# ruchikachavhan/diffusion-models-moe

Hardware: AMD Instinct MI355X
Metric: images/sec SD-1.4 512² 50-step DDIM, expert mask on; 1→8 GPU scaling (higher is better)
Workload: dtype fp16; 1 GPU; SD-1.4 MoE-fied (relu, top-k 0.2, expert 20) + RemoveExperts skilled-expert mask, 512^2 (4x64x64 latents), 50 DDIM steps, CFG 7.5; prompts_per_gpu=8, global_batch=8, parallelism=dp1

## Files before the change

diffusion-models-moe_amd/sdmoe/_lib.py:

```python
from __future__ import annotations

import ctypes
import os

_HERE = os.path.dirname(os.path.abspath(__file__))
LIB_PATH = os.path.join(_HERE, "libsdmoe_hip.so")

_P = ctypes.c_void_p
_L = ctypes.c_long
_I = ctypes.c_int
_F = ctypes.c_float
_FP = ctypes.POINTER(ctypes.c_float)
_IP = ctypes.POINTER(ctypes.c_int)

SIGNATURES = {
    "sdmoe_linear": [_P, _L, _P, _L, _P, _P, _L, _I, _P, _L, _P, _L, _I, _I, _I, _I, _P, _L, _P],
    "sdmoe_conv3x3": [_P, _L, _I, _I, _I, _I, _P, _P, _P, _L, _P, _L, _P, _L, _I, _I, _I, _I, _P, _L, _P],
    "sdmoe_conv3x3_sc": [_P, _L, _I, _I, _I, _I, _P, _P, _P, _L, _P, _L, _I, _P, _L, _I, _I, _P, _L, _P],
    "sdmoe_conv3x3_gn": [_P, _L, _I, _I, _I, _I, _P, _P, _I, _P, _P, _P, _L, _P, _L, _P, _L, _I, _P, _L, _I, _P, _L,
                         _P],
    "sdmoe_conv_up2x": [_P, _L, _I, _I, _I, _I, _P, _P, _P, _L, _I, _P, _L, _P],
    "sdmoe_conv_up2x_plan": [_I, _I, _I, _I, _I, _L, _P],
    "sdmoe_groupnorm_apply": [_P, _L, _I, _I, _I, _P, _P, _I, _P, _L, _P],
    "sdmoe_mask_weight": [_P, _P, _L, _L, _P, _P],
    "sdmoe_groupnorm_stats": [_P, _L, _I, _I, _I, _I, _P, _P, _F, _P, _P, _P, _L, _P],
    "sdmoe_groupnorm": [_P, _L, _I, _I, _I, _I, _P, _P, _F, _I, _P, _L, _P, _P, _P, _L, _P],
    "sdmoe_gn_fold": [_P, _L, _I, _I, _P, _P, _P, _I, _P, _P, _P],
    "sdmoe_linear_per_image": [_P, _L, _P, _L, _L, _P, _L, _I, _P, _L, _P, _L, _I, _I, _I, _P, _L, _P],
    "sdmoe_layernorm": [_P, _L, _P, _L, _I, _I, _P, _P, _F, _P],
    "sdmoe_ln_fold": [_P, _L, _I, _I, _P, _P, _P, _P, _L, _P, _P, _P],
    "sdmoe_linear_ln": [_P, _L, _P, _L, _P, _P, _F, _P, _L, _I, _I, _I, _P],
    "sdmoe_linear_geglu_ln": [_P, _L, _P, _L, _P, _P, _F, _P, _L, _I, _I, _I, _I, _P, _L, _I, _P],
    "sdmoe_attention": [_P, _L, _P, _L, _P, _L, _P, _L, _I, _I, _I, _I, _I, _F, _P],
    "sdmoe_geglu_route": [_P, _L, _I, _I, _I, _I, _I, _P, _P, _P, _P, _P, _L, _P, _L, _P, _P, _P],
    "sdmoe_score_bias": [_P, _L, _I, _I, _P, _P, _L, _P],
    "sdmoe_geglu_route_bias": [_P, _L, _I, _I, _I, _I, _I, _P, _P, _P, _P, _P, _L, _P, _L, _P, _P, _P, _P],
    "sdmoe_linear_geglu": [_P, _L, _P, _L, _P, _P, _L, _I, _I, _I, _I, _P, _L, _I, _P],
    "sdmoe_moe_topk_mask": [_P, _L, _I, _I, _I, _I, _I, _P, _L, _P, _P, _P],
    "sdmoe_moe_topk_keep": [_I, _I, _I, _I, _I, _P, _L, _P, _P, _P, _P],
    "sdmoe_linear_keep": [_P, _L, _P, _P, _L, _P, _P, _L, _P, _L, _I, _I, _I, _P, _L, _P],
    "sdmoe_linear_masked": [_P, _L, _P, _P, _L, _P, _P, _P, _L, _P, _L, _I, _I, _I, _P, _L, _P],
    "sdmoe_linear_masked_sets": [_P, _L, _P, _P, _L, _P, _L, _P, _I, _I, _P, _P, _L, _P, _L, _I, _I, _I, _P, _L, _P],
    "sdmoe_gemm_plan_sets": [_I, _I, _I, _I, _I, _I, _L, _P],
    "sdmoe_wmask_union_sets": [_P, _L, _I, _P, _I, _L, _P, _P],
    "sdmoe_gemm_plan": [_I, _I, _I, _I, _I, _I, _L, _P],
    "sdmoe_conv_plan": [_I, _I, _I, _I, _I, _I, _I, _I, _I, _I, _I, _L, _P],
    "sdmoe_wmask_kmajor": [_P, _L, _I, _I, _P, _P, _P],
    "sdmoe_timestep_embedding": [_P, _P, _F, _I, _I, _F, _P],
    "sdmoe_cfg_multistep_step": [_P, _L, _P, _I, _I, _I, _F, _P, _P, _P, _P, _P, _L, _P],
    "sdmoe_sqdist_f32": [_P, _L, _P, _L, _I, _I, _I, _P, _L, _P],
    "sdmoe_balanced_assign": [_P, _I, _I, ctypes.c_double, _P, _I, _P],
    "sdmoe_expert_mean_topk": [_P, _L, _I, _I, _I, _P, _I, _I, _P, _P, _P, _L, _P],
    "sdmoe_colnorm_accum": [_P, _L, _I, _I, _P, _P, _L, _P],
    "sdmoe_wanda_mask": [_P, _L, _I, _I, _P, _P, _I, _P, _P],
    "sdmoe_union_over_time": [_P, _L, _I, _L, _F, _P, _P],
    "sdmoe_geglu_neurons": [_P, _L, _I, _I, _I, _P, _F, _P, _L, _P, _L, _I, _P, _I, _P, _P, _P, _L, _P],
    "sdmoe_expert_stats": [_P, _L, _P, _I, _I, _I, _P, _I, _P, _P, _P, _L, _P],
    "sdmoe_geglu_sparsity": [_P, _L, _I, _I, _I, _F, _P, _L, _P, _L, _I, _P, _I, _P, _P, _P, _P, _L, _P],
    "sdmoe_noise_capture": [_P, _L, _P, _L, _L, _P],
    "sdmoe_noise_distance": [_P, _L, _L, _P, _L, _L, _I, _I, _I, _P, _I, _P, _P, _L, _P],
    "sdmoe_clip_quantise": [_P, _I, _I, _I, _I, _P, _P],
    "sdmoe_clip_resample_h": [_P, _L, _I, _I, _I, _I, _I, _P, _P, _I, _I, _P, _P],
    "sdmoe_clip_resample_v": [_P, _I, _I, _I, _P, _P, _I, _I, _I, _FP, _FP, _P, _P, _L, _I, _P],
    "sdmoe_clip_scores": [_P, _L, _P, _L, _P, _L, _I, _I, _P, _P],
    "sdmoe_text_pool": [_P, _L, _I, _I, _I, _I, _I, _P, _L, _P],
    "sdmoe_concept_route": [_P, _L, _I, _I, _I, _P, _L, _I, _P, _P, _I, _P, _P, _P, _P],
    "sdmoe_softmax_rows": [_P, _L, _P, _L, _I, _I, _P],
    "sdmoe_transpose": [_P, _L, _P, _L, _I, _I, _P],
    "sdmoe_gather_rows": [_P, _L, _P, _I, _I, _P, _L, _I, _P, _L, _P],
    "sdmoe_attention_short": [_P, _L, _P, _L, _P, _L, _P, _L, _I, _I, _I, _I, _F, _I, _P],
    "sdmoe_timestep_embedding_rows": [_P, _L, _P, _I, _I, _I, _I, _F, _P],
    "sdmoe_prepare_input": [_P, _P, _I, _I, _L, _I, _P],
    "sdmoe_cfg_ddim_step": [_P, _L, _P, _I, _I, _I, _F, _F, _F, _P, _L, _P],
    "sdmoe_cfg_x0_step": [_P, _L, _P, _I, _I, _I, _F, _P, _P, _P, _P, _L, _P],
    "sdmoe_prepare_input_scaled": [_P, _P, _I, _I, _L, _I, _F, _F, _P],
    "sdmoe_add": [_P, _P, _P, _L, _P],
    "sdmoe_tune": [_I, _I],
    "sdmoe_tune_knob": [_I, _IP, ctypes.POINTER(ctypes.c_char_p), _IP, _IP],
    "sdmoe_tune_reset": [],
    "sdmoe_set_gelu_table": [_P],
    "sdmoe_version": [],
}

ERRORS = {-1: "bad pointer/size", -2: "unsupported shape/alignment", -3: "unsupported mode"}

_lib = None


class SdmoeError(RuntimeError):
    pass


def load(path: str | None = None):
    global _lib
    if _lib is not None:
        return _lib
    p = path or os.environ.get("SDMOE_LIB", LIB_PATH)
    if not os.path.exists(p):
        raise SdmoeError(
            f"libsdmoe_hip.so not found at {p}: build it with `python -c 'import __graft_entry__ as g; g.build()'` "
            "(or `make -C diffusion-models-moe_amd/csrc`). There is no CPU fallback."
        )
    lib = ctypes.CDLL(p)
    ab_lib = os.environ.get("SDMOE_AB", "0") == "1"
    for name, argt in SIGNATURES.items():
        if ab_lib and not hasattr(lib, name):
            continue
        fn = getattr(lib, name)
        fn.argtypes = argt
        fn.restype = ctypes.c_char_p if name == "sdmoe_version" else ctypes.c_int
    for k, v in parse_tune(os.environ.get("SDMOE_TUNE", ""), lib):
        check(lib.sdmoe_tune(k, v), f"sdmoe_tune({k}={v})")
    _lib = lib
    return lib

# ... 42 lines not shown
```

diffusion-models-moe_amd/sdmoe/ops.py:

```python
from __future__ import annotations

import ctypes
import os

import torch

from . import _lib

ACT_NONE, ACT_SILU, ACT_GELU, ACT_RELU, ACT_QUICK_GELU = 0, 1, 2, 3, 4
ACT_BY_NAME = {"none": ACT_NONE, "silu": ACT_SILU, "gelu": ACT_GELU, "relu": ACT_RELU, "quick_gelu": ACT_QUICK_GELU}


_raw_stream = getattr(torch._C, "_cuda_getCurrentRawStream", None)
_cur_dev = getattr(torch._C, "_cuda_getDevice", None)


def _stream():
    if _raw_stream is not None and _cur_dev is not None:
        return _raw_stream(_cur_dev())
    return torch.cuda.current_stream().cuda_stream


def _ptr(t):
    return None if t is None else t.data_ptr()
# ... 492 lines not shown
    lib = _lib.load()
    xp, lda = _rows(x, "x")
    M, K = x.shape
    nimg, N, Kw = wf.shape
    if Kw != K or M != nimg * rows_per_batch or tuple(colbias.shape) != (nimg, N):
        raise ValueError(f"linear_per_image: x {tuple(x.shape)}, wf {tuple(wf.shape)}, colbias "
                         f"{tuple(colbias.shape)}, rows_per_batch {rows_per_batch}")
    if out is None:
        out = torch.empty((M, N), dtype=torch.float16, device=x.device)
    op, ldc = _rows(out, "out")
    rp, ldr = (None, 0) if residual is None else _rows(residual, "residual")
    ws = _workspace(x.device)
    st = lib.sdmoe_linear_per_image(xp, lda, _dev(wf, "wf"), wf.stride(1), wf.stride(0),
                                    _dev(colbias, "colbias", torch.float32), colbias.stride(0), rows_per_batch, rp,
                                    ldr, op, ldc, M, N, K, ws.data_ptr(), ws.numel(), _stream())
    _lib.check(st, "sdmoe_linear_per_image")
    return out


def layernorm(x, gamma, beta, eps=1e-5, out=None):
    lib = _lib.load()
    xp, ldx = _rows(x, "x")
    M, C = x.shape
    if out is None:
        out = torch.empty((M, C), dtype=torch.float16, device=x.device)
    op, ldy = _rows(out, "out")
    st = lib.sdmoe_layernorm(xp, ldx, op, ldy, M, C, _dev(gamma, "gamma"), _dev(beta, "beta"), float(eps), _stream())
    _lib.check(st, "sdmoe_layernorm")
    return out


class LNFold:

    def __init__(self, w, gamma, beta, eps, bias=None):
        lib = _lib.load()
        N, K = w.shape
        self.eps = float(eps)
        self.w = torch.empty((N, K), dtype=torch.float16, device=w.device)
        self.bias = torch.empty(N, dtype=torch.float32, device=w.device)
        self.wsum = torch.empty(N, dtype=torch.float32, device=w.device)
        if bias is not None:
            _dev(bias, "bias")
        st = lib.sdmoe_ln_fold(_dev(w, "w"), w.stride(0), N, K, _dev(gamma, "gamma"), _dev(beta, "beta"), _ptr(bias),
                               self.w.data_ptr(), K, self.bias.data_ptr(), self.wsum.data_ptr(), _stream())
        _lib.check(st, "sdmoe_ln_fold")

    def rows(self, idx):
        f = LNFold.__new__(LNFold)
        f.eps, f.w, f.bias, f.wsum = self.eps, self.w[idx].contiguous(), self.bias[idx].contiguous(), \
            self.wsum[idx].contiguous()
        return f


def linear_ln(x, fold: LNFold, out=None):
    lib = _lib.load()
    xp, lda = _rows(x, "x")
    M, K = x.shape
    N = fold.w.shape[0]
    if fold.w.shape[1] != K:
        raise ValueError(f"linear_ln: folded weight {tuple(fold.w.shape)} does not match input K={K}")
    if out is None:
        out = torch.empty((M, N), dtype=torch.float16, device=x.device)
    op, ldc = _rows(out, "out")
    st = lib.sdmoe_linear_ln(xp, lda, fold.w.data_ptr(), fold.w.stride(0), fold.bias.data_ptr(), fold.wsum.data_ptr(),
                             fold.eps, op, ldc, M, N, K, _stream())
    _lib.check(st, "sdmoe_linear_ln")
    return out


def attention(q, k, v, nimg, Nq, Nk, heads, out=None, scale=None):
    lib = _lib.load()
    qp, ldq = _rows(q, "q")
    kp, ldk = _rows(k, "k")
    vp, ldv = _rows(v, "v")
    C = q.shape[1]
    d = C // heads
    if out is None:
        out = torch.empty((nimg * Nq, C), dtype=torch.float16, device=q.device)
    op, ldo = _rows(out, "out")
    if scale is None:
        scale = d ** -0.5
    st = lib.sdmoe_attention(qp, ldq, kp, ldk, vp, ldv, op, ldo, nimg, Nq, Nk, heads, d, float(scale), _stream())
    _lib.check(st, "sdmoe_attention")
    return out


class Routing:

    def __init__(self, labels: torch.Tensor, num_experts: int, k: int, device):
        labels = labels.to(torch.int64).cpu()
        F = labels.numel()
        if labels.min() < 0 or labels.max() >= num_experts:
            raise ValueError("expert labels out of range")
        order = torch.argsort(labels, stable=True)
        counts = torch.bincount(labels, minlength=num_experts)
        off = torch.zeros(num_experts + 1, dtype=torch.int64)
        off[1:] = torch.cumsum(counts, 0)
        self.F, self.E, self.k = F, int(num_experts), int(k)
        self.labels = labels.to(torch.int32).to(device)
        self.e_off = off.to(torch.int32).to(device)
        self.e_nid = order.to(torch.int32).to(device)
        sizes = set(counts.tolist())
        self.esize = sizes.pop() if len(sizes) == 1 else 0
        self.perm = order
        self.perm_dev = order.to(torch.int32).to(device)
        self.fusable = bool(self.esize and 40 % self.esize == 0 and F % 80 == 0 and self.E <= 256)

    @classmethod
    def from_patterns(cls, patterns: torch.Tensor, k: int, device=None):
        p = patterns.detach().float().cpu()
        E, F = p.shape
        if not torch.all((p == 0) | (p == 1)) or not torch.all(p.sum(0) == 1):
            raise ValueError("patterns must be a 0/1 [E, F] matrix with exactly one expert per neuron")
        labels = p.argmax(0)
        return cls(labels, E, k, device or patterns.device)


def geglu_rows(F: int, perm: torch.Tensor | None, device) -> torch.Tensor:
    if F % 2:
        raise ValueError(f"GEGLU layout: F = {F} is odd")
    idx = torch.arange(F, device=device) if perm is None else perm.to(device)
    r = torch.arange(2 * F, device=device)
    q, e = r // 4, r % 4
    c = 2 * q + (e & 1)
    return torch.where(e < 2, idx[c], F + idx[c])


def interleave_geglu(weight: torch.Tensor, bias: torch.Tensor | None, perm: torch.Tensor | None):
    F2, K = weight.shape
    rows = geglu_rows(F2 // 2, perm, weight.device)
    b = torch.zeros(F2, dtype=weight.dtype, device=weight.device) if bias is None else bias
    return weight[rows].contiguous(), b[rows].contiguous()


def interleave_ln_fold(fold: LNFold, perm: torch.Tensor | None) -> LNFold:
    F = fold.w.shape[0] // 2
    return fold.rows(geglu_rows(F, perm, fold.w.device))


_GELU_TABLES = {}


def gelu_table_values() -> torch.Tensor:
    i = torch.arange(16384, dtype=torch.int32)
    bits = (0x2800 + (i & 8191)) | ((i >> 13) << 15)
    return bits.to(torch.int16).view(torch.float16)


def ensure_gelu_table(device) -> torch.Tensor:
    dev = torch.device(device)
    idx = dev.index if dev.index is not None else torch.cuda.current_device()
    t = _GELU_TABLES.get(idx)
    if t is None:
        t = torch.nn.functional.gelu(gelu_table_values().to(torch.device("cuda", idx))).contiguous()
        lib = _lib.load()
        if _lib.has(lib, "sdmoe_set_gelu_table"):
            with torch.cuda.device(idx):
                _lib.check(lib.sdmoe_set_gelu_table(t.data_ptr()), "sdmoe_set_gelu_table")
        _GELU_TABLES[idx] = t
    return t


def linear_geglu(x, w_il, b_il, act=ACT_GELU, *, score=None, esize=0, out=None, ln: LNFold | None = None):
    lib = _lib.load()
    if act == ACT_GELU:
        ensure_gelu_table(x.device)
# ... 762 lines not shown
```

diffusion-models-moe_amd/sdmoe/unet.py:

```python
from __future__ import annotations

import os

import torch
import torch.nn as nn
import torch.nn.functional as F

from . import ops
from .config import UNetConfig

CTX_LEN = 77
FUSED_GEGLU = True
FUSED_KEEP = True
FUSED_LN = os.environ.get("SDMOE_FUSED_LN", "1") != "0"
FUSED_LN_FFN = os.environ.get("SDMOE_FUSED_LN_FFN", "0") == "1"
FUSED_SC = os.environ.get("SDMOE_FUSED_SC", "1") != "0"
FUSED_GN = os.environ.get("SDMOE_FUSED_GN", "1") != "0"
GN_FOLD_MIN_HW = 1024
UPCONV_COLLAPSE = os.environ.get("SDMOE_UPCONV_COLLAPSE", "1") != "0"
IN_PAD = 64
OUT_PAD = 8


def _buf(t):
    return nn.Parameter(t, requires_grad=False)


class LoRACompatibleLinear(nn.Module):

    def __init__(self, weight, bias=None):
        super().__init__()
        self.weight = _buf(weight)
        self.bias = None if bias is None else _buf(bias)
        self._sdmoe_deferred = 0

    @property
    def in_features(self):
        return self.weight.shape[1]

    @property
    def out_features(self):
        return self.weight.shape[0]

    def run(self, x2d, weight=None, **kw):
        return ops.linear(x2d, self.weight if weight is None else weight, self.bias, **kw)

    def forward(self, x, scale=1.0):
        if self._sdmoe_deferred and self._forward_hooks:
            return None
        shp = x.shape
        return self.run(x.reshape(-1, shp[-1])).view(*shp[:-1], self.out_features)


class Conv2d(nn.Module):

    def __init__(self, weight, bias, stride=1):
        super().__init__()
        self.weight = _buf(weight)
        self.bias = _buf(bias)
        self.stride = stride


class Norm(nn.Module):
    def __init__(self, weight, bias, eps, groups=None):
        super().__init__()
        self.weight = _buf(weight)
        self.bias = _buf(bias)
        self.eps = eps
        self.groups = groups

    def stats(self, x2d, nimg, HW):
        return ops.groupnorm_stats(x2d, nimg, HW, self.weight, self.bias, self.eps, self.groups)

    def normalize(self, x2d, nimg, HW, silu):
        return ops.groupnorm(x2d, nimg, HW, self.weight, self.bias, self.eps, self.groups, silu)


def act_code(fn):
    from_name = getattr(fn, "_sdmoe_act", None)
    if from_name is not None:
        return ops.ACT_BY_NAME[from_name]
    if fn is F.gelu or fn is torch.nn.functional.gelu:
        return ops.ACT_GELU
    if fn is F.relu or fn is torch.relu:
        return ops.ACT_RELU
    raise NotImplementedError(f"GEGLU activation {fn!r} has no HIP kernel (supported: gelu, relu)")


def _gelu(x):
    return F.gelu(x)


_gelu._sdmoe_act = "gelu"


class GEGLU(nn.Module):

    def __init__(self, proj: LoRACompatibleLinear):
        super().__init__()
        self.proj = proj
        self.gelu = _gelu
        self.patterns = None
# ... 150 lines not shown
        return view(out), view(gate)

    def sparsity(self, x, threshold=0.0, col_zero=None, col_neg=None, totals=None, img_group=None, ngroups=1,
                 want_gate=False):
        y, rpi, gate, view = self._seam_operands(x, want_gate)
        out = ops.geglu_sparsity(y, act_code(self.gelu), threshold=threshold, rows_per_img=rpi, img_group=img_group,
                                 ngroups=ngroups, col_zero=col_zero, col_neg=col_neg, totals=totals, gate_out=gate)
        return view(out), view(gate)

    def forward(self, x, scale=1.0):
        if self._sdmoe_deferred and self._forward_hooks:
            return None
        return self.routed(x)[0]


def _sole_receiver(module, method):
    hooks = list(module._forward_hooks.values())
    if len(hooks) != 1:
        return None
    owner = getattr(hooks[0], "__self__", None)
    if owner is None or not getattr(owner, "_sdmoe_receiver", False) or not hasattr(owner, method):
        return None
    return owner


def _ln_safe_hook(module, owner):
    if owner is None:
        return False
    hooks = list(module._forward_hooks.values())
    fn = getattr(hooks[0], "__func__", None) if len(hooks) == 1 else None
    return fn is not None and fn is getattr(type(owner), "_sdmoe_ln_safe_hook", None)


class FeedForward(nn.Module):
    def __init__(self, geglu, down):
        super().__init__()
        self.net = nn.ModuleList([geglu, nn.Dropout(0.0), down])
        self._wperm_key = None
        self._wperm = None

    def _down_weight_permuted(self, routing):
        w = self.net[2].weight
        key = (id(routing), w.data_ptr(), w._version)
        if self._wperm_key != key:
            self._wperm = w.data[:, routing.perm.to(w.device)].contiguous()
            self._wperm_key = key
        return self._wperm

    def run(self, x2d, nimg, residual, ln=None):
        geglu, down = self.net[0], self.net[2]
        dhooks = bool(down._forward_hooks)
        masker = _sole_receiver(down, "fused_linear") if dhooks else None
        owner = _sole_receiver(geglu, "hook_fn") if geglu._forward_hooks else None
        geglu._allow_permuted_out = (not dhooks or masker is not None) and (not geglu._forward_hooks or owner is not None)
        if ln is not None and geglu._forward_hooks and not _ln_safe_hook(geglu, owner):
            x2d = ops.layernorm(x2d, ln.weight, ln.bias, ln.eps)
            ln = None
        xv = x2d.view(nimg, -1, x2d.shape[1])
        geglu._ln_pending = (xv, ln) if ln is not None else None
        try:
            h = geglu(xv)
        finally:
            geglu._allow_permuted_out = False
            geglu._ln_pending = None
        h2 = h.reshape(-1, h.shape[-1])
        perm = geglu._out_perm
        permuted = perm is not None and perm[1] == h2.data_ptr()
        if dhooks and not (permuted and masker is not None):
            o = down(h)
            return ops.add(o.reshape(residual.shape).contiguous(), residual)
        if permuted:
            wp = self._down_weight_permuted(perm[0])
            keep = geglu._out_keep
            keep = keep[0] if keep is not None and keep[1] == h2.data_ptr() else None
            if masker is not None:
                kw = {"nimg": nimg} if getattr(masker, "_sdmoe_fused_nimg", False) else {}
                return masker.fused_linear(down, h2, keep, perm[0].perm_dev, wp, residual, **kw)
            if keep is not None:
                return ops.linear_keep(h2, keep, wp, down.bias, residual=residual)
            return ops.linear(h2, wp, down.bias, residual=residual)
        return down.run(h2, residual=residual)


class Attention(nn.Module):
    def __init__(self, wq, wk, wv, wo, bo, heads, self_attn):
        super().__init__()
        self.heads = heads
        self.self_attn = self_attn
        C = wq.shape[0]
        if self_attn:
            self.w_qkv = _buf(torch.cat([wq, wk, wv], 0).contiguous())
            self.to_q = LoRACompatibleLinear(self.w_qkv.data[:C])
            self.to_k = LoRACompatibleLinear(self.w_qkv.data[C:2 * C])
            self.to_v = LoRACompatibleLinear(self.w_qkv.data[2 * C:])
        else:
            self.w_kv = _buf(torch.cat([wk, wv], 0).contiguous())
            self.to_q = LoRACompatibleLinear(wq)
            self.to_k = LoRACompatibleLinear(self.w_kv.data[:C])
            self.to_v = LoRACompatibleLinear(self.w_kv.data[C:])
        self.to_out = nn.ModuleList([LoRACompatibleLinear(wo, bo), nn.Dropout(0.0)])
        self._kv_key = None
        self._kv = None
        self._ln_key = None
        self._ln_fold = None

    def _fold(self, norm):
        w = self.w_qkv if self.self_attn else self.to_q.weight
        key = (w.data_ptr(), w._version, norm.weight.data_ptr(), norm.weight._version, norm.bias.data_ptr(),
               norm.bias._version)
        if self._ln_key != key:
            self._ln_fold = ops.LNFold(w.data, norm.weight.data, norm.bias.data, norm.eps)
            self._ln_key = key
        return self._ln_fold

    def cross_kv(self, ctx2d):
        key = (ctx2d, ctx2d._version, self.w_kv.data_ptr(), self.w_kv._version)
        k = self._kv_key
        if k is None or k[0] is not ctx2d or k[1:] != key[1:]:
            self._kv = ops.linear(ctx2d, self.w_kv)
            self._kv_key = key
        return self._kv

    def run(self, x2d, nimg, N, residual, ctx2d=None, ln=None):
        C = x2d.shape[1]
        if self.self_attn:
            qkv = ops.linear(x2d, self.w_qkv) if ln is None else ops.linear_ln(x2d, self._fold(ln))
            a = ops.attention(qkv[:, :C], qkv[:, C:2 * C], qkv[:, 2 * C:], nimg, N, N, self.heads)
        else:
            q = ops.linear(x2d, self.to_q.weight) if ln is None else ops.linear_ln(x2d, self._fold(ln))
            kv = self.cross_kv(ctx2d)
            a = ops.attention(q, kv[:, :C], kv[:, C:], nimg, N, ctx2d.shape[0] // nimg, self.heads)
        return self.to_out[0].run(a, residual=residual)


class BasicTransformerBlock(nn.Module):
    def __init__(self, norm1, attn1, norm2, attn2, norm3, ff):
        super().__init__()
        self.norm1, self.attn1, self.norm2, self.attn2, self.norm3, self.ff = norm1, attn1, norm2, attn2, norm3, ff

    def run(self, hs, nimg, N, ctx2d):
        if FUSED_LN and hs.shape[1] % 64 == 0:
            hs = self.attn1.run(hs, nimg, N, residual=hs, ln=self.norm1)
            hs = self.attn2.run(hs, nimg, N, residual=hs, ctx2d=ctx2d, ln=self.norm2)
            if FUSED_LN_FFN:
                return self.ff.run(hs, nimg, residual=hs, ln=self.norm3)
            n = ops.layernorm(hs, self.norm3.weight, self.norm3.bias, self.norm3.eps)
            return self.ff.run(n, nimg, residual=hs)
        n = ops.layernorm(hs, self.norm1.weight, self.norm1.bias, self.norm1.eps)
        hs = self.attn1.run(n, nimg, N, residual=hs)
        n = ops.layernorm(hs, self.norm2.weight, self.norm2.bias, self.norm2.eps)
        hs = self.attn2.run(n, nimg, N, residual=hs, ctx2d=ctx2d)
        n = ops.layernorm(hs, self.norm3.weight, self.norm3.bias, self.norm3.eps)
        return self.ff.run(n, nimg, residual=hs)


class Transformer2DModel(nn.Module):

    def __init__(self, norm, proj_in, blocks, proj_out):
        super().__init__()
        self.norm = norm
        self.proj_in = proj_in
        self.transformer_blocks = nn.ModuleList(blocks)
        self.proj_out = proj_out

    def run(self, x, nimg, HW, ctx2d, out):
        pi = self.proj_in
        if FUSED_GN and HW >= GN_FOLD_MIN_HW and HW % 256 == 0 and x.shape[1] % 64 == 0 and not pi._forward_hooks:
            scale, shift = self.norm.stats(x, nimg, HW)
            wf, cb = ops.gn_fold(pi.weight, pi.bias, scale, shift)
            hs = ops.linear_per_image(x, wf, cb, HW)
        else:
            hs = pi.run(self.norm.normalize(x, nimg, HW, False))
        for blk in self.transformer_blocks:
            hs = blk.run(hs, nimg, HW, ctx2d)
        return self.proj_out.run(hs, residual=x, out=out)


class ResnetBlock2D(nn.Module):
    def __init__(self, norm1, conv1, temb_proj, norm2, conv2, shortcut):
        super().__init__()
        self.norm1, self.conv1, self.time_emb_proj, self.norm2, self.conv2 = norm1, conv1, temb_proj, norm2, conv2
        self.conv_shortcut = shortcut
        self.temb_slice = None
        self._sc_key = None
        self._sc_w = None

    def _conv2_with_shortcut(self):
        w2, b2, ws, bs = self.conv2.weight, self.conv2.bias, self.conv_shortcut.weight, self.conv_shortcut.bias
        key = tuple(None if t is None else (t.data_ptr(), t._version) for t in (w2, b2, ws, bs))
        if self._sc_key != key:
            b = sum(t.data.float() for t in (b2, bs) if t is not None)
            self._sc_w = (ops.conv_weight_with_shortcut(w2.data, ws.data),
                          None if isinstance(b, int) else b.half())
            self._sc_key = key
        return self._sc_w

    def run(self, x, nimg, H, W, temb_all, out):
        HW = H * W
        o, n = self.temb_slice
        bstride = temb_all.stride(0) if temb_all.shape[0] > 1 else 0
        cmid = self.conv1.weight.shape[0]
        if ops.conv_gn_fusable(H, W, x.shape[1], cmid):
            h = ops.conv3x3(x, nimg, H, W, self.conv1.weight, self.conv1.bias, coladd=temb_all[:, o:o + n],
                            coladd_bstride=bstride, gn=self.norm1.stats(x, nimg, HW) + (True,))
        else:
            xn = self.norm1.normalize(x, nimg, HW, True)
            h = ops.conv3x3(xn, nimg, H, W, self.conv1.weight, self.conv1.bias,
                            coladd=temb_all[:, o:o + n], coladd_bstride=bstride)
        gn2 = None
        hn = h
        if ops.conv_gn_fusable(H, W, cmid, self.conv2.weight.shape[0]):
            gn2 = self.norm2.stats(h, nimg, HW) + (True,)
        else:
# ... 297 lines not shown
```

include/sdmoe.h:

```cpp
#ifndef SDMOE_H
#define SDMOE_H

#ifdef __cplusplus
extern "C" {
#endif

#define SDMOE_ACT_NONE 0
#define SDMOE_ACT_SILU 1
#define SDMOE_ACT_GELU 2
#define SDMOE_ACT_RELU 3
#define SDMOE_ACT_QUICK_GELU 4

const char* sdmoe_version(void);

int sdmoe_linear(const void* A, long lda, const void* W, long ldw, const void* bias, const void* coladd,
                 long coladd_bstride, int rows_per_batch, const void* R, long ldr, void* C, long ldc, int M, int N,
                 int K, int act, float* workspace, long workspace_floats, void* stream);

int sdmoe_conv3x3(const void* X, long ldx, int nimg, int H, int W, int Cin, const void* Wt, const void* bias,
                  const void* coladd, long coladd_bstride, const void* R, long ldr, void* Y, long ldy, int Cout,
                  int stride, int upsample, int act, float* workspace, long workspace_floats, void* stream);

int sdmoe_conv3x3_sc(const void* X, long ldx, int nimg, int H, int W, int Cin, const void* Wt, const void* bias,
                     const void* coladd, long coladd_bstride, const void* X2, long ldx2, int Cin2, void* Y, long ldy,
                     int Cout, int act, float* workspace, long workspace_floats, void* stream);

int sdmoe_conv3x3_gn(const void* X, long ldx, int nimg, int H, int W, int Cin, const float* gn_scale,
                     const float* gn_shift, int silu, const void* Wt, const void* bias, const void* coladd,
                     long coladd_bstride, const void* R, long ldr, const void* X2, long ldx2, int Cin2, void* Y,
                     long ldy, int Cout, float* workspace, long workspace_floats, void* stream);

int sdmoe_conv_up2x(const void* X, long ldx, int nimg, int H, int W, int Cin, const void* Wc, const void* bias, void* Y,
                    long ldy, int Cout, float* workspace, long workspace_floats, void* stream);
int sdmoe_conv_up2x_plan(int nimg, int H, int W, int Cin, int Cout, long workspace_floats, int* out);

int sdmoe_groupnorm_apply(const void* X, long ldx, int nimg, int HW, int C, const float* scale, const float* shift,
                          int silu, void* Y, long ldy, void* stream);

int sdmoe_mask_weight(const void* W, const void* bits, long N, long K, void* Wm, void* stream);

int sdmoe_groupnorm_stats(const void* X, long ldx, int nimg, int HW, int C, int groups, const void* gamma,
                          const void* beta, float eps, float* scale, float* shift, float* workspace,
                          long workspace_floats, void* stream);

int sdmoe_groupnorm(const void* X, long ldx, int nimg, int HW, int C, int groups, const void* gamma, const void* beta,
                    float eps, int silu, void* Y, long ldy, float* scale, float* shift, float* workspace,
                    long workspace_floats, void* stream);

int sdmoe_gn_fold(const void* W, long ldw, int N, int K, const void* bias, const float* scale, const float* shift,
                  int nimg, void* Wf, float* colbias, void* stream);
int sdmoe_linear_per_image(const void* A, long lda, const void* Wf, long ldw, long w_bstride, const float* colbias,
                           long colbias_bstride, int rows_per_batch, const void* R, long ldr, void* C, long ldc, int M,
                           int N, int K, float* workspace, long workspace_floats, void* stream);

int sdmoe_layernorm(const void* X, long ldx, void* Y, long ldy, int M, int C, const void* gamma, const void* beta,
                    float eps, void* stream);

int sdmoe_ln_fold(const void* W, long ldw, int N, int K, const void* gamma, const void* beta, const void* bias,
                  void* Wf, long ldf, float* bias_f, float* wsum, void* stream);
int sdmoe_linear_ln(const void* A, long lda, const void* Wf, long ldw, const float* bias_f, const float* wsum,
                    float eps, void* C, long ldc, int M, int N, int K, void* stream);
int sdmoe_linear_geglu_ln(const void* A, long lda, const void* W, long ldw, const float* bias_f, const float* wsum,
                          float eps, void* P, long ldp, int M, int F, int K, int act, void* score, long ld_score,
                          int esize, void* stream);

int sdmoe_attention(const void* Q, long ldq, const void* K, long ldk, const void* V, long ldv, void* O, long ldo,
                    int nimg, int Nq, int Nk, int heads, int head_dim, float scale, void* stream);

int sdmoe_geglu_route(const void* Y, long ldy, int M, int F, int E, int k, int act, const int* labels,
                      const int* e_off, const int* e_nid, const unsigned* removed_bits, void* out, long ldo,
                      void* gate_out, long ldg, unsigned* sel_out, void* score_out, void* stream);

int sdmoe_score_bias(const void* score, long ld_score, int M, int E, const void* bias, void* out, long ld_out,
                     void* stream);
int sdmoe_geglu_route_bias(const void* Y, long ldy, int M, int F, int E, int k, int act, const int* labels,
                           const int* e_off, const int* e_nid, const unsigned* removed_bits, void* out, long ldo,
                           void* gate_out, long ldg, unsigned* sel_out, void* score_out, const void* bias,
                           void* stream);

int sdmoe_linear_geglu(const void* A, long lda, const void* W, long ldw, const void* bias, void* P, long ldp,
                       int M, int F, int K, int act, void* score, long ld_score, int esize, void* stream);
int sdmoe_moe_topk_mask(void* P, long ldp, int M, int F, int E, int esize, int k, const void* score,
                        long ld_score, const unsigned* removed_bits, unsigned* sel_out, void* stream);

int sdmoe_moe_topk_keep(int M, int F, int E, int esize, int k, const void* score, long ld_score,
                        const unsigned* removed_bits, void* keep, unsigned* sel_out, void* stream);
int sdmoe_linear_keep(const void* A, long lda, const void* keep, const void* W, long ldw, const void* bias,
                      const void* R, long ldr, void* C, long ldc, int M, int N, int K, float* workspace,
                      long workspace_floats, void* stream);

int sdmoe_linear_masked(const void* A, long lda, const void* keep, const void* W, long ldw, const void* wmask,
                        const void* bias, const void* R, long ldr, void* C, long ldc, int M, int N, int K,
                        float* workspace, long workspace_floats, void* stream);

int sdmoe_linear_masked_sets(const void* A, long lda, const void* keep, const void* W, long ldw, const void* wmasks,
                             long set_stride, const int* image_set, int nsets, int rows_per_img, const void* bias,
                             const void* R, long ldr, void* C, long ldc, int M, int N, int K, float* workspace,
                             long workspace_floats, void* stream);

int sdmoe_gemm_plan_sets(int has_keep, int M, int N, int K, int rows_per_img, int has_residual, long workspace_floats,
                         int* out);

int sdmoe_wmask_union_sets(const void* masks, long mask_stride, int nconcepts, const unsigned* select, int nsets,
                           long words, void* out, void* stream);

int sdmoe_gemm_plan(int mode, int M, int N, int K, int has_residual, int act, long workspace_floats, int* out);

int sdmoe_conv_plan(int nimg, int H, int W, int Cin, int Cin2, int Cout, int stride, int upsample, int has_residual,
                    int gn, int act, long workspace_floats, int* out);

int sdmoe_wmask_kmajor(const void* bits, long ldb, int N, int K, const int* perm, void* out, void* stream);

int sdmoe_expert_mean_topk(const void* score, long ld_score, int M, int E, int rows_per_img, const int* row_idx,
                           int n_idx, int k, void* mean_out, int* topk_out, float* workspace, long workspace_floats,
                           void* stream);
int sdmoe_expert_stats(const void* score, long ld_score, const unsigned* sel, int M, int E, int rows_per_img,
                       const int* img_group, int ngroups, void* colmax, int* count, float* workspace,
                       long workspace_floats, void* stream);
int sdmoe_colnorm_accum(const void* P, long ldp, int M, int F, float* sumsq, float* workspace, long workspace_floats,
                        void* stream);
int sdmoe_wanda_mask(const void* W, long ldw, int C, int F, const void* norm_base, const void* norm_adj, int kprune,
                     void* bits, void* stream);

int sdmoe_geglu_neurons(const void* Y, long ldy, int M, int F, int act, const unsigned* override_bits,
                        float override_value, void* out, long ldo, void* gate_out, long ldg, int rows_per_img,
                        const int* img_group, int ngroups, const unsigned* pos_bits, void* colmax, float* workspace,
                        long workspace_floats, void* stream);

int sdmoe_geglu_sparsity(const void* Y, long ldy, int M, int F, int act, float threshold, void* out, long ldo,
                         void* gate_out, long ldg, int rows_per_img, const int* img_group, int ngroups, int* col_zero,
                         int* col_neg, int64_t* totals, float* workspace, long workspace_floats, void* stream);

int sdmoe_sqdist_f32(const float* X, long ldx, const float* C, long ldc, int n, int k, int d, float* D, long ldd,
                     void* stream);
int sdmoe_balanced_assign(const double* cost, int n, int k, double scale, int64_t* prices, int warm, int* labels);

int sdmoe_union_over_time(const void* bits, long t_stride_bytes, int T, long nbytes, float threshold, void* out,
                          void* stream);

int sdmoe_softmax_rows(const void* X, long ldx, void* Y, long ldy, int R, int N, void* stream);
int sdmoe_transpose(const void* X, long ldx, void* Y, long ldy, int R, int C, void* stream);

int sdmoe_gather_rows(const void* table, long ld_table, const int* idx, int R, int C, const void* add, long ld_add,
                      int period, void* out, long ld_out, void* stream);
int sdmoe_attention_short(const void* Q, long ldq, const void* K, long ldk, const void* V, long ldv, void* O,
                          long ldo, int nseq, int N, int heads, int head_dim, float scale, int causal, void* stream);

int sdmoe_timestep_embedding(void* out, const float* t_dev, float t, int dim, int flip_sin_to_cos, float freq_shift,
                             void* stream);
int sdmoe_timestep_embedding_rows(void* out, long ldo, const float* t_dev, int n, int group, int dim,
// ... 58 lines not shown
```

Baseline: 9.810 images/s.

## Fuse LN-folded Q projection, cross-attention and output projection into one kernel

Adds a single HIP kernel for the C=320, 8-head cross-attention block. Each 128-row tile computes the LayerNorm statistics, the folded Q GEMM, per-head attention over up to 96 keys, the output projection with bias, and the residual add, all kept in LDS. Weight slabs and K/V are triple/double-buffered through LDS with async buffer loads. This removes the Q and attention-output round trips through global memory and two extra launches. The cost is heavy LDS use that allows only one block per CU, and the path is limited to one specific shape with a fallback to the old path otherwise.

```diff
diff --git a/diffusion-models-moe_amd/csrc/xattn_block.hip b/diffusion-models-moe_amd/csrc/xattn_block.hip
--- /dev/null
+++ b/diffusion-models-moe_amd/csrc/xattn_block.hip
@@ -0,0 +1,385 @@
+#include <type_traits>
+
+#include "common.h"
+#include "../../include/sdmoe.h"
+
+namespace {
+
+constexpr int C = 320, HEADS = 8, D = 40;
+constexpr int BM = 128, NW = 8, NT = NW * 64;
+constexpr int XRS = 336;
+constexpr int KSTEP = 32, NKS = C / KSTEP;
+constexpr int SLAB = C * KSTEP;
+constexpr int NPIECE = SLAB * 2 / 1024;
+constexpr int MAXK = 96;
+constexpr int KVROWS = 128;
+constexpr int RS = 48, SL = RS / 8, CH = D / 8;
+constexpr int KVT = KVROWS * RS;
+constexpr int KVPIECE = KVT * 2 / 1024;
+constexpr int SLOT = 2 * KVT;
+constexpr unsigned OOB = 0x80000000u;
+static_assert(2 * KVPIECE == 3 * NW, "three K/V pieces per wave and head");
+static_assert(SLAB <= SLOT, "a slab fits a ring slot");
+
+struct XParams {
+  const half_t* x; long ldx;
+  const half_t* wq; long ldwq; const float* bq; const float* wsum; float eps;
+  const half_t* K; long ldk; const half_t* V; long ldv; int Nk;
+  const half_t* wo; long ldwo; const half_t* bo;
+  half_t* out; long ldo;
+  int Nq;
+  float scale_log2;
+};
+
+SDMOE_DEV half4 ds_read_tr(const half_t* p) {
+  typedef short s4 __attribute__((ext_vector_type(4)));
+  s4 v = __builtin_amdgcn_ds_read_tr16_b64_v4i16((s4 __attribute__((address_space(3)))*)(p));
+  return __builtin_bit_cast(half4, v);
+}
+
+SDMOE_DEV float max3(float a, float b, float c) { return fmaxf(fmaxf(a, b), c); }
+SDMOE_DEV float max2(float a, float b) { return fmaxf(a, b); }
+SDMOE_DEV float max_xrows(float v) {
+  auto r = __builtin_amdgcn_permlane32_swap(__float_as_uint(v), __float_as_uint(v), false, false);
+  v = max2(__uint_as_float(r[0]), __uint_as_float(r[1]));
+  auto t = __builtin_amdgcn_permlane16_swap(__float_as_uint(v), __float_as_uint(v), false, false);
+  return max2(__uint_as_float(t[0]), __uint_as_float(t[1]));
+}
+
+typedef __attribute__((address_space(3))) void lds_void_t;
+SDMOE_DEV void bld16(__amdgpu_buffer_rsrc_t rs, const half_t* lds_dst, unsigned voff) {
+  __builtin_amdgcn_raw_ptr_buffer_load_lds(rs, (lds_void_t*)lds_dst, 16, voff, 0, 0, 0);
+}
+template <int N>
+SDMOE_DEV void vm_wait() { asm volatile("s_waitcnt vmcnt(%0)" ::"n"(N) : "memory"); }
+SDMOE_DEV void barrier() {
+  __builtin_amdgcn_s_barrier();
+  asm volatile("" ::: "memory");
+}
+
+SDMOE_DEV int swz(int t) { return (0x78 >> (2 * t)) & 3; }
+
+__global__ __launch_bounds__(NT, 1) void xattn_block_kernel(XParams p) {
+  __shared__ __attribute__((aligned(1024))) half_t XT[BM * XRS];
+  __shared__ __attribute__((aligned(1024))) half_t R0[SLOT];
+  __shared__ __attribute__((aligned(1024))) half_t R1[SLOT];
+  __shared__ __attribute__((aligned(1024))) half_t R2[SLOT];
+  __shared__ __attribute__((aligned(1024))) half_t ONES[16 * 16];
+  __shared__ float LNROW[BM * 2];
+
+  const int tid = threadIdx.x, lane = tid & 63;
+  const int wave = __builtin_amdgcn_readfirstlane(tid >> 6);
+  const int g = lane >> 4, w = lane & 15;
+  const int wr = wave >> 2, wc = wave & 3;
+  const int tile = xcd_remap(blockIdx.x, gridDim.x);
+  const long row0 = (long)tile * BM;
+  const int img = (int)(row0 / p.Nq);
+
+  const __amdgpu_buffer_rsrc_t rsWq = __builtin_amdgcn_make_buffer_rsrc(
+      (void*)p.wq, (short)0, (int)((C - 1) * p.ldwq * 2 + C * 2), 0x00020000);
+  const __amdgpu_buffer_rsrc_t rsWo = __builtin_amdgcn_make_buffer_rsrc(
+      (void*)p.wo, (short)0, (int)((C - 1) * p.ldwo * 2 + C * 2), 0x00020000);
+  const __amdgpu_buffer_rsrc_t rsK = __builtin_amdgcn_make_buffer_rsrc(
+      (void*)(p.K + (long)img * p.Nk * p.ldk), (short)0, (int)(((long)p.Nk - 1) * p.ldk * 2 + C * 2), 0x00020000);
+  const __amdgpu_buffer_rsrc_t rsV = __builtin_amdgcn_make_buffer_rsrc(
+      (void*)(p.V + (long)img * p.Nk * p.ldv), (short)0, (int)(((long)p.Nk - 1) * p.ldv * 2 + C * 2), 0x00020000);
+
+  auto slot_at = [&](int i) -> half_t* { return i == 0 ? R0 : (i == 1 ? R1 : R2); };
+
+  const int wrow = lane >> 2, wchunk = (lane & 3) ^ swz((lane >> 4) & 3);
+  auto issue_slab = [&](__amdgpu_buffer_rsrc_t rs, long ldw, int ks, half_t* dst) {
+#pragma unroll
+    for (int j = 0; j < 3; ++j) {
+      const int pc = wave + NW * j;
+      if (j < 2 || wave < NPIECE - 2 * NW)
+        bld16(rs, dst + pc * 512, (unsigned)((16 * pc + wrow) * ldw * 2 + wchunk * 16 + ks * (KSTEP * 2)));
+    }
+  };
+
+  float4v acc[4][5];
+  const int aoff = w * KSTEP + ((g ^ swz((w >> 2) & 3)) << 3);
+  auto tile_gemm = [&](__amdgpu_buffer_rsrc_t rs, long ldw) {
+#pragma unroll
+    for (int i = 0; i < 4; ++i)
+#pragma unroll
+      for (int j = 0; j < 5; ++j) acc[i][j] = (float4v){0.f, 0.f, 0.f, 0.f};
+#pragma unroll
+    for (int s = 0; s < NKS; ++s) {
+      if (s + 1 < NKS) {
+        if (wave < NPIECE - 2 * NW) vm_wait<3>();
+        else vm_wait<2>();
+      } else {
+        vm_wait<0>();
+      }
+      barrier();
+      if (s + 2 < NKS) issue_slab(rs, ldw, s + 2, slot_at((s + 2) % 3));
+      const half_t* Ws = slot_at(s % 3) + wc * 80 * KSTEP + aoff;
+      const half_t* Xs = XT + (wr * 64 + w) * XRS + KSTEP * s + 8 * g;
+      half8 bf[4], af[5];
+#pragma unroll
+      for (int i = 0; i < 4; ++i) bf[i] = *reinterpret_cast<const half8*>(Xs + 16 * i * XRS);
+#pragma unroll
+      for (int j = 0; j < 5; ++j) af[j] = *reinterpret_cast<const half8*>(Ws + 16 * j * KSTEP);
+#pragma unroll
+      for (int i = 0; i < 4; ++i)
+#pragma unroll
+        for (int j = 0; j < 5; ++j) acc[i][j] = mfma16x16x32(af[j], bf[i], acc[i][j]);
+    }
+  };
+
+  issue_slab(rsWq, p.ldwq, 0, R0);
+  issue_slab(rsWq, p.ldwq, 1, R1);
+  for (int i = tid; i < 16 * 16; i += NT) ONES[i] = (half_t)(i % 16 == 8 ? 1.f : 0.f);
+  const int crow = tid >> 3, cch = tid & 7;
+  {
+    typedef _Float16 h2 __attribute__((ext_vector_type(2)));
+    const h2 one2 = {(half_t)1.f, (half_t)1.f};
+    half8 xr[2][5];
+#pragma unroll
+    for (int h = 0; h < 2; ++h)
+#pragma unroll
+      for (int i = 0; i < 5; ++i)
+        xr[h][i] = *reinterpret_cast<const half8*>(p.x + (row0 + crow + 64 * h) * p.ldx + (cch + 8 * i) * 8);
+#pragma unroll
+    for (int h = 0; h < 2; ++h) {
+      float s1 = 0.f, s2 = 0.f;
+#pragma unroll
+      for (int i = 0; i < 5; ++i) {
+#pragma unroll
+        for (int q = 0; q < 4; ++q) {
+          const h2 x2 = {xr[h][i][2 * q], xr[h][i][2 * q + 1]};
+          s1 = __builtin_amdgcn_fdot2(x2, one2, s1, false);
+          s2 = __builtin_amdgcn_fdot2(x2, x2, s2, false);
+        }
+        *reinterpret_cast<half8*>(XT + (crow + 64 * h) * XRS + (cch + 8 * i) * 8) = xr[h][i];
+      }
+#pragma unroll
+      for (int o = 1; o < 8; o <<= 1) {
+        s1 += __shfl_xor(s1, o, 64);
+        s2 += __shfl_xor(s2, o, 64);
+      }
+      if (cch == 0) {
+        const float mean = s1 / (float)C;
+        const float var = fmaxf(s2 / (float)C - mean * mean, 0.f);
+        const float rstd = rsqrtf(var + p.eps);
+        LNROW[2 * (crow + 64 * h)] = rstd;
+        LNROW[2 * (crow + 64 * h) + 1] = -mean * rstd;
+      }
+    }
+  }
+  __syncthreads();
+
+  tile_gemm(rsWq, p.ldwq);
+
+  unsigned kvoff[3];
+  int kvlds[3];
+#pragma unroll
+  for (int j = 0; j < 3; ++j) {
+    const int gp = wave + NW * j;
+    const bool isk = gp < KVPIECE;
+    const int pc = isk ? gp : gp - KVPIECE;
+    const int slot = pc * 64 + lane, r = slot / SL, c = slot - (slot / SL) * SL;
+    const long ld = isk ? p.ldk : p.ldv;
+    kvoff[j] = c < CH ? (unsigned)(r * ld * 2 + c * 16) : OOB;
+    kvlds[j] = (isk ? 0 : KVT) + pc * 512;
+  }
+  auto issue_kv = [&](int h, half_t* dst) {
+#pragma unroll
+    for (int j = 0; j < 3; ++j)
+      bld16(wave + NW * j < KVPIECE ? rsK : rsV, dst + kvlds[j], kvoff[j] + (unsigned)(h * D * 2));
+  };
+
+  {
+    float4v ws[5], lb[5];
+#pragma unroll
+    for (int j = 0; j < 5; ++j) {
+      const int n = wc * 80 + 16 * j + 4 * g;
+      ws[j] = *reinterpret_cast<const float4v*>(p.wsum + n);
+      lb[j] = *reinterpret_cast<const float4v*>(p.bq + n);
+    }
+    __syncthreads();
+    issue_kv(0, R0);
+#pragma unroll
+    for (int i = 0; i < 4; ++i) {
+      const int m = wr * 64 + 16 * i + w;
+      const float a = LNROW[2 * m], c = LNROW[2 * m + 1];
+#pragma unroll
+      for (int j = 0; j < 5; ++j) {
+        half4 y;
+#pragma unroll
+        for (int r = 0; r < 4; ++r)
+          y[r] = (half_t)__builtin_fmaf(a, acc[i][j][r], __builtin_fmaf(c, ws[j][r], lb[j][r]));
+        *reinterpret_cast<half4*>(XT + m * XRS + wc * 80 + 16 * j + 4 * g) = y;
+      }
+    }
+  }
+
+  {
+    half_t* Xw = XT + (wave * 16 + w) * XRS;
+    const int tq = w >> 2, tp = w & 3;
+    auto head = [&](int h, auto buf_tag) {
+      constexpr int BUF = decltype(buf_tag)::value;
+      const half_t* Kt = BUF ? R1 : R0;
+      const half_t* Vt = Kt + KVT;
+      vm_wait<0>();
+      asm volatile("s_waitcnt lgkmcnt(0)" ::: "memory");
+      barrier();
+      if (h + 1 < HEADS) issue_kv(h + 1, BUF ? R0 : R1);
+
+      half8 qf[2];
+#pragma unroll
+      for (int c = 0; c < 2; ++c) {
+        const int d = 32 * c + 8 * g;
+        half8 v = {0, 0, 0, 0, 0, 0, 0, 0};
+        if (d < D) v = *reinterpret_cast<const half8*>(Xw + h * D + d);
+#pragma unroll
+        for (int j = 0; j < 8; ++j) v[j] = (half_t)((float)v[j] * p.scale_log2);
+        qf[c] = v;
+      }
+      float4v s[6];
+#pragma unroll
+      for (int kf = 0; kf < 6; ++kf) {
+        s[kf] = (float4v){0.f, 0.f, 0.f, 0.f};
+#pragma unroll
+        for (int c = 0; c < 2; ++c) {
+          const half8 a = *reinterpret_cast<const half8*>(Kt + (kf * 16 + w) * RS + 32 * c + 8 * g);
+          s[kf] = mfma16x16x32(a, qf[c], s[kf]);
+        }
+      }
+#pragma unroll
+      for (int kf = 0; kf < 6; ++kf)
+#pragma unroll
+        for (int i = 0; i < 4; ++i)
+          if (kf * 16 + 4 * g + i >= p.Nk) s[kf][i] = -INFINITY;
+      float m0 = max3(s[0][0], s[0][1], s[0][2]);
+      float m1 = max3(s[0][3], s[1][0], s[1][1]);
+      float m2 = max3(s[1][2], s[1][3], s[2][0]);
+      float m3 = max3(s[2][1], s[2][2], s[2][3]);
+      float m4 = max3(s[3][0], s[3][1], s[3][2]);
+      float m5 = max3(s[3][3], s[4][0], s[4][1]);
+      float m6 = max3(s[4][2], s[4][3], s[5][0]);
+      float m7 = max3(s[5][1], s[5][2], s[5][3]);
+      m0 = max3(m0, m1, m2);
+      m3 = max3(m3, m4, m5);
+      m6 = max3(m6, m7, m0);
+      const float mx = max_xrows(max2(m3, m6));
+      half8 pb[3];
+#pragma unroll
+      for (int c2 = 0; c2 < 3; ++c2) {
+        half8 v;
+#pragma unroll
+        for (int i = 0; i < 4; ++i) {
+          v[i] = (half_t)__builtin_amdgcn_exp2f(s[2 * c2][i] - mx);
+          v[4 + i] = (half_t)__builtin_amdgcn_exp2f(s[2 * c2 + 1][i] - mx);
+        }
+        pb[c2] = v;
+      }
+      float4v oacc[3];
+#pragma unroll
+      for (int df = 0; df < 3; ++df) oacc[df] = (float4v){0.f, 0.f, 0.f, 0.f};
+#pragma unroll
+      for (int c2 = 0; c2 < 3; ++c2)
+#pragma unroll
+        for (int df = 0; df < 3; ++df) {
+          const half_t* a0 = Vt + (32 * c2 + 4 * g + tq) * RS + 16 * df + 4 * tp;
+          const half_t* a1 = a0 + 16 * RS;
+          if (df == D / 16 && 4 * tp == D % 16) a0 = a1 = ONES + (4 * g + tq) * 16 + 8;
+          const half4 lo = ds_read_tr(a0), hi = ds_read_tr(a1);
+          const half8 a = {lo[0], lo[1], lo[2], lo[3], hi[0], hi[1], hi[2], hi[3]};
+          oacc[df] = mfma16x16x32(a, pb[c2], oacc[df]);
+        }
+      const float l = __shfl(oacc[D / 16][D % 4], ((D % 16) / 4) * 16 + w, 64);
+      const float inv = 1.0f / l;
+#pragma unroll
+      for (int df = 0; df < 3; ++df) {
+        const int d = 16 * df + 4 * g;
+        if (d < D) {
+          half4 o;
+#pragma unroll
+          for (int i = 0; i < 4; ++i) o[i] = (half_t)(oacc[df][i] * inv);
+          *reinterpret_cast<half4*>(Xw + h * D + d) = o;
+        }
+      }
+    };
+    for (int h = 0; h < HEADS; h += 2) {
+      head(h, std::integral_constant<int, 0>());
+      head(h + 1, std::integral_constant<int, 1>());
+    }
+  }
+
+  __syncthreads();
+  issue_slab(rsWo, p.ldwo, 0, R0);
+  issue_slab(rsWo, p.ldwo, 1, R1);
+  tile_gemm(rsWo, p.ldwo);
+  {
+    half4 b4[5];
+#pragma unroll
+    for (int j = 0; j < 5; ++j)
+      b4[j] = p.bo ? *reinterpret_cast<const half4*>(p.bo + wc * 80 + 16 * j + 4 * g) : (half4){0, 0, 0, 0};
+    __syncthreads();
+#pragma unroll
+    for (int i = 0; i < 4; ++i) {
+      const int m = wr * 64 + 16 * i + w;
+#pragma unroll
+      for (int j = 0; j < 5; ++j) {
+        half4 y;
+#pragma unroll
+        for (int r = 0; r < 4; ++r) y[r] = (half_t)(acc[i][j][r] + (float)b4[j][r]);
+        *reinterpret_cast<half4*>(XT + m * XRS + wc * 80 + 16 * j + 4 * g) = y;
+      }
+    }
+  }
+  half8 xr[2][5];
+#pragma unroll
+  for (int h = 0; h < 2; ++h)
+#pragma unroll
+    for (int i = 0; i < 5; ++i)
+      xr[h][i] = *reinterpret_cast<const half8*>(p.x + (row0 + crow + 64 * h) * p.ldx + (cch + 8 * i) * 8);
+  __syncthreads();
+#pragma unroll
+  for (int h = 0; h < 2; ++h)
+#pragma unroll
+    for (int i = 0; i < 5; ++i) {
+      half8 o = *reinterpret_cast<const half8*>(XT + (crow + 64 * h) * XRS + (cch + 8 * i) * 8);
+#pragma unroll
+      for (int j = 0; j < 8; ++j) o[j] = (half_t)((float)o[j] + (float)xr[h][i][j]);
+      *reinterpret_cast<half8*>(p.out + (row0 + crow + 64 * h) * p.ldo + (cch + 8 * i) * 8) = o;
+    }
+}
+
+bool overlaps(const void* a, long abytes, const void* b, long bbytes) {
+  const char* pa = (const char*)a;
+  const char* pb = (const char*)b;
+  return pa < pb + bbytes && pb < pa + abytes;
+}
+
+}
+
+extern "C" int sdmoe_cross_attn_block(const void* x, long ldx, const void* wq_f, long ldwq, const float* bq_f,
+                                      const float* wq_sum, float eps, const void* K, long ldk, const void* V, long ldv,
+                                      int Nk, const void* wo, long ldwo, const void* bo, void* out, long ldo, int nimg,
+                                      int Nq, int heads, int head_dim, float scale, void* stream) {
+  if (!x || !wq_f || !bq_f || !wq_sum || !K || !V || !wo || !out || nimg < 0 || Nq < 0 || Nk <= 0 || heads <= 0 ||
+      head_dim <= 0)
+    return SDMOE_EARG;
+  if (heads != HEADS || head_dim != D || Nk > MAXK || Nq % BM) return SDMOE_EUNSUP;
+  if (ldx % 8 || ldo % 8 || ldk % 8 || ldv % 8 || ldwq % 8 || ldwo % 8 || ldx < C || ldo < C || ldk < C || ldv < C ||
+      ldwq < C || ldwo < C)
+    return SDMOE_ESHAPE;
+  if (((uintptr_t)x | (uintptr_t)out | (uintptr_t)K | (uintptr_t)V | (uintptr_t)wq_f | (uintptr_t)wo |
+       (uintptr_t)bq_f | (uintptr_t)wq_sum) % 16 || (uintptr_t)bo % 8)
+    return SDMOE_ESHAPE;
+  if ((long)Nk * ldk * 2 >= (1L << 31) || (long)Nk * ldv * 2 >= (1L << 31) || C * ldwq * 2 >= (1L << 31) ||
+      C * ldwo * 2 >= (1L << 31))
+    return SDMOE_EUNSUP;
+  const long M = (long)nimg * Nq;
+  if (M == 0) return SDMOE_OK;
+  if (M / BM >= (1L << 31)) return SDMOE_EUNSUP;
+  if (overlaps(x, ((M - 1) * ldx + C) * 2, out, ((M - 1) * ldo + C) * 2)) return SDMOE_EUNSUP;
+  XParams p{(const half_t*)x, ldx, (const half_t*)wq_f, ldwq, bq_f, wq_sum, eps, (const half_t*)K, ldk,
+            (const half_t*)V, ldv, Nk, (const half_t*)wo, ldwo, (const half_t*)bo, (half_t*)out, ldo, Nq,
+            scale * 1.4426950408889634f};
+  xattn_block_kernel<<<dim3((unsigned)(M / BM)), NT, 0, (hipStream_t)stream>>>(p);
+  SDMOE_CHECK_LAUNCH();
+  return SDMOE_OK;
+}
diff --git a/diffusion-models-moe_amd/sdmoe/_lib.py b/diffusion-models-moe_amd/sdmoe/_lib.py
--- a/diffusion-models-moe_amd/sdmoe/_lib.py
+++ b/diffusion-models-moe_amd/sdmoe/_lib.py
@@ -31,6 +31,8 @@
     "sdmoe_ln_fold": [_P, _L, _I, _I, _P, _P, _P, _P, _L, _P, _P, _P],
     "sdmoe_linear_ln": [_P, _L, _P, _L, _P, _P, _F, _P, _L, _I, _I, _I, _P],
     "sdmoe_linear_geglu_ln": [_P, _L, _P, _L, _P, _P, _F, _P, _L, _I, _I, _I, _I, _P, _L, _I, _P],
+    "sdmoe_cross_attn_block": [_P, _L, _P, _L, _P, _P, _F, _P, _L, _P, _L, _I, _P, _L, _P, _P, _L, _I, _I, _I, _I, _F,
+                               _P],
     "sdmoe_attention": [_P, _L, _P, _L, _P, _L, _P, _L, _I, _I, _I, _I, _I, _F, _P],
     "sdmoe_geglu_route": [_P, _L, _I, _I, _I, _I, _I, _P, _P, _P, _P, _P, _L, _P, _L, _P, _P, _P],
     "sdmoe_score_bias": [_P, _L, _I, _I, _P, _P, _L, _P],
diff --git a/diffusion-models-moe_amd/sdmoe/ops.py b/diffusion-models-moe_amd/sdmoe/ops.py
--- a/diffusion-models-moe_amd/sdmoe/ops.py
+++ b/diffusion-models-moe_amd/sdmoe/ops.py
@@ -598,6 +598,41 @@
         scale = d ** -0.5
     st = lib.sdmoe_attention(qp, ldq, kp, ldk, vp, ldv, op, ldo, nimg, Nq, Nk, heads, d, float(scale), _stream())
     _lib.check(st, "sdmoe_attention")
+    return out
+
+
+XATTN_BLOCK_ROWS = 128
+XATTN_BLOCK_MAX_KEYS = 96
+
+
+def cross_attn_block_supported(C, heads, Nk, Nq):
+    return (C == 320 and heads == 8 and 1 <= Nk <= XATTN_BLOCK_MAX_KEYS and Nq > 0
+            and Nq % XATTN_BLOCK_ROWS == 0)
+
+
+def cross_attn_block(x, fold: LNFold, k, v, wo, bo, nimg, Nq, Nk, heads, out=None, scale=None):
+    lib = _lib.load()
+    xp, ldx = _rows(x, "x")
+    kp, ldk = _rows(k, "k")
+    vp, ldv = _rows(v, "v")
+    C = x.shape[1]
+    if x.shape[0] != nimg * Nq or k.shape[0] != nimg * Nk or v.shape[0] != nimg * Nk:
+        raise ValueError("cross_attn_block: rows do not match nimg*Nq / nimg*Nk")
+    if tuple(fold.w.shape) != (C, C) or tuple(wo.shape) != (C, C) or k.shape[1] != C or v.shape[1] != C:
+        raise ValueError(f"cross_attn_block: operands do not match C={C}")
+    d = C // heads
+    if out is None:
+        out = torch.empty((x.shape[0], C), dtype=torch.float16, device=x.device)
+    op, ldo = _rows(out, "out")
+    if scale is None:
+        scale = d ** -0.5
+    st = lib.sdmoe_cross_attn_block(xp, ldx, fold.w.data_ptr(), fold.w.stride(0), fold.bias.data_ptr(),
+                                    fold.wsum.data_ptr(), fold.eps, kp, ldk, vp, ldv, Nk, _dev(wo, "wo"), wo.stride(0),
+                                    None if bo is None else _dev(bo, "bo"), op, ldo, nimg, Nq, heads, d, float(scale),
+                                    _stream())
+    if st == -3:
+        return None
+    _lib.check(st, "sdmoe_cross_attn_block")
     return out
 
 
diff --git a/diffusion-models-moe_amd/sdmoe/unet.py b/diffusion-models-moe_amd/sdmoe/unet.py
--- a/diffusion-models-moe_amd/sdmoe/unet.py
+++ b/diffusion-models-moe_amd/sdmoe/unet.py
@@ -6,7 +6,7 @@
 import torch.nn as nn
 import torch.nn.functional as F
 
-from . import ops
+from . import _lib, ops
 from .config import UNetConfig
 
 CTX_LEN = 77
@@ -18,6 +18,8 @@
 FUSED_GN = os.environ.get("SDMOE_FUSED_GN", "1") != "0"
 GN_FOLD_MIN_HW = 1024
 UPCONV_COLLAPSE = os.environ.get("SDMOE_UPCONV_COLLAPSE", "1") != "0"
+XATTN_FUSED = os.environ.get("SDMOE_XATTN_FUSED", "1") != "0"
+XATTN_MIN_TILES = 256
 IN_PAD = 64
 OUT_PAD = 8
 
@@ -334,6 +336,12 @@
         return down.run(h2, residual=residual)
 
 
+def xattn_fused_rule(C, heads, nimg, Nq, Nk, has_kernel=True):
+    if not has_kernel or not ops.cross_attn_block_supported(C, heads, Nk, Nq):
+        return False
+    return nimg * Nq // ops.XATTN_BLOCK_ROWS >= XATTN_MIN_TILES
+
+
 class Attention(nn.Module):
     def __init__(self, wq, wk, wv, wo, bo, heads, self_attn):
         super().__init__()
@@ -373,14 +381,26 @@
             self._kv_key = key
         return self._kv
 
+    def cross_fused(self, C, nimg, N, Nk):
+        if self.self_attn or not XATTN_FUSED:
+            return False
+        return xattn_fused_rule(C, self.heads, nimg, N, Nk, _lib.has(_lib.load(), "sdmoe_cross_attn_block"))
+
     def run(self, x2d, nimg, N, residual, ctx2d=None, ln=None):
         C = x2d.shape[1]
         if self.self_attn:
             qkv = ops.linear(x2d, self.w_qkv) if ln is None else ops.linear_ln(x2d, self._fold(ln))
             a = ops.attention(qkv[:, :C], qkv[:, C:2 * C], qkv[:, 2 * C:], nimg, N, N, self.heads)
         else:
+            kv = self.cross_kv(ctx2d)
+            Nk = ctx2d.shape[0] // nimg
+            if ln is not None and residual is x2d and self.cross_fused(C, nimg, N, Nk):
+                to_out = self.to_out[0]
+                o = ops.cross_attn_block(x2d, self._fold(ln), kv[:, :C], kv[:, C:], to_out.weight, to_out.bias, nimg,
+                                         N, Nk, self.heads)
+                if o is not None:
+                    return o
             q = ops.linear(x2d, self.to_q.weight) if ln is None else ops.linear_ln(x2d, self._fold(ln))
-            kv = self.cross_kv(ctx2d)
             a = ops.attention(q, kv[:, :C], kv[:, C:], nimg, N, ctx2d.shape[0] // nimg, self.heads)
         return self.to_out[0].run(a, residual=residual)
 
diff --git a/include/sdmoe.h b/include/sdmoe.h
--- a/include/sdmoe.h
+++ b/include/sdmoe.h
@@ -66,6 +66,11 @@
 
 int sdmoe_attention(const void* Q, long ldq, const void* K, long ldk, const void* V, long ldv, void* O, long ldo,
                     int nimg, int Nq, int Nk, int heads, int head_dim, float scale, void* stream);
+
+int sdmoe_cross_attn_block(const void* x, long ldx, const void* wq_f, long ldwq, const float* bq_f,
+                           const float* wq_sum, float eps, const void* K, long ldk, const void* V, long ldv, int Nk,
+                           const void* wo, long ldwo, const void* bo, void* out, long ldo, int nimg, int Nq,
+                           int heads, int head_dim, float scale, void* stream);
 
 int sdmoe_geglu_route(const void* Y, long ldy, int M, int F, int E, int k, int act, const int* labels,
                       const int* e_off, const int* e_nid, const unsigned* removed_bits, void* out, long ldo,
```

Result: no change. 9.859 images/s, median of 6 (+0.5%).
